# dell-research-harvard/effocr

Hardware: AMD Instinct MI355X
Metric: glyph-crops/sec end-to-end (encode+kNN), 224x224 bs=1024 (higher is better)
Workload: dtype bf16; 1 GPU; BASELINE configs[1]: vit_small_patch16_224 encoder (bf16 MFMA operands, fp32 accumulate/residual/LN/softmax), 1024x3x224x224 fp32 crops per GPU resident in HBM, 10000-row fp32 IndexFlatIP, k=10; seeded random-init weights; crops_per_gpu=1024, global_batch=1024, index_rows=10000, k=10, parallelism=1024 crops per GPU, weights+index replicated

## Files before the change

effocr_amd/csrc/qkvattn.hip:

```cpp
#include "common.hpp"
#include "kernels.hpp"
#include <math.h>
#include <type_traits>

#ifndef QA_NT
#define QA_NT 0
#endif
#ifndef QA_ODD_TILE_WAVE
#define QA_ODD_TILE_WAVE 1
#endif
#ifndef QA_BARRIER_DRAIN
#define QA_BARRIER_DRAIN 0
#endif
#ifndef QA_EDGE_BLOCK_MAJOR
#define QA_EDGE_BLOCK_MAJOR 1
#endif

namespace effocr {
namespace {

#ifdef QA_STAMP
constexpr int QA_STAMP_WGS = 256, QA_STAMP_N = 16;
__device__ unsigned long long qa_stamps[QA_STAMP_WGS * 4 * QA_STAMP_N];
#define QA_STAMP_AT(k) qa_stamps[((blockIdx.x & (QA_STAMP_WGS - 1)) * 4 + w) * QA_STAMP_N + (k)] = __builtin_amdgcn_s_memtime();
#else
#define QA_STAMP_AT(k)
#endif

template <int I, int N, typename F> __device__ __forceinline__ void qa_for(F&& f) {
  if constexpr (I < N) {
    f(std::integral_constant<int, I>{});
    qa_for<I + 1, N>(f);
  }
}


constexpr int QA_STAGE = 16384;
constexpr int QA_RING = 6;

template <typename E, int D, int NTT, bool CLS = false, int NPV = 2 * NTT>
__global__ __launch_bounds__(256, 1) void qkvattn_kernel(QkvAttnArgs a) {
  typedef typename Op16<E>::V8 V8;
  constexpr int HEADS = D / 64;
  constexpr int KC = D / 8;
  constexpr int KT = D / 128;
  constexpr int NSH = 3 * KT;
  constexpr int NS = HEADS * NSH;
  constexpr int NXF = D / 16;
  constexpr int R = QA_RING;
  constexpr bool SMALL = NSH < R - 1;
  static_assert(D % 128 == 0 && NS >= R - 1, "qkvattn: embed dim must be a multiple of 128");
  __shared__ __attribute__((aligned(16))) char smem[R * QA_STAGE + NTT * 8192 + 3 * D * 4];
  char* sK = smem;
  char* sV = sK + NTT * 4096;
  float* sBias = reinterpret_cast<float*>(sV + NTT * 4096);
  char* sW = smem + NTT * 8192 + 3 * D * 4;

  const int tid = threadIdx.x;
  int lane = tid & 63, r31 = lane & 31, half = lane >> 5;
  auto refresh_lane = [&]() __attribute__((always_inline)) {
    asm volatile("" : "+v"(lane));
    r31 = lane & 31;
    half = lane >> 5;
  };
  const int w = wave_id();
  QA_STAMP_AT(14)
  const int T = a.T;
  int64_t tok0 = 0;
  const int HS = a.hsplit > 1 ? a.hsplit : 1, NH = HEADS / HS;
  const int grp = (int)blockIdx.x % HS, slot0 = a.img0 + (int)blockIdx.x / HS, nslots = (int)gridDim.x / HS;
  const int hb = grp * NH;
  const int h0 = ((int)blockIdx.x >> 3) % NH;
  const char* Wb = static_cast<const char*>(a.Wb);

  {
    const unsigned sB_lds = (unsigned)(size_t)(__attribute__((address_space(3))) char*)sBias;
#pragma unroll
    for (int j = 0; j < (3 * D / 4 + 255) / 256; ++j) {
      const int u = j * 256 + tid;
      const char* src = reinterpret_cast<const char*>(a.bias) + (size_t)u * 16;
      const unsigned dst = (unsigned)__builtin_amdgcn_readfirstlane((int)(sB_lds + (unsigned)(j * 256 + (tid >> 6) * 64) * 16u));
      if (u < 3 * D / 4)
        asm volatile("s_mov_b32 m0, %1\n\t"
                     "s_nop 0\n\t"
                     "global_load_lds_dwordx4 %0, off"
                     :: "v"(src), "s"(dst) : "memory", "m0");
    }
  }

  int ih = hb + h0, isec = 0, ikt = 0, islot = 0;
  const unsigned lane16 = (unsigned)(tid & 63) * 16u;
  auto issue_piece = [&](int p) __attribute__((always_inline)) {
    const int rb = (isec * D + ih * 64) / 32 + (w >> 1);
    const __attribute__((address_space(1))) void* src =
        (const __attribute__((address_space(1))) void*)(Wb + ((size_t)rb * KC + ikt * 16 + (w & 1) * 8) * 512 + lane16);
    __attribute__((address_space(3))) void* dst = (__attribute__((address_space(3))) void*)(sW + islot * QA_STAGE + ((w >> 1) * 16 + (w & 1) * 8) * 512);
    switch (p) {
      case 0: __builtin_amdgcn_global_load_lds(src, dst, 16, 0, 0); break;
      case 1: __builtin_amdgcn_global_load_lds(src, dst, 16, 1024, 0); break;
      case 2: __builtin_amdgcn_global_load_lds(src, dst, 16, 2048, 0); break;
      default: __builtin_amdgcn_global_load_lds(src, dst, 16, 3072, 0); break;
    }
  };
  const unsigned sW_lds = (unsigned)(size_t)(__attribute__((address_space(3))) char*)sW;
  auto issue_piece_asm = [&](auto P_) __attribute__((always_inline)) {
    constexpr int pc = decltype(P_)::value;
    const int rb = (isec * D + ih * 64) / 32 + (w >> 1);
    const char* src = Wb + ((size_t)rb * KC + ikt * 16 + (w & 1) * 8) * 512 + lane16;
    const unsigned dst = (unsigned)__builtin_amdgcn_readfirstlane((int)(sW_lds + (unsigned)(islot * QA_STAGE) + (unsigned)(((w >> 1) * 16 + (w & 1) * 8) * 512)));
    unsigned keep;
    asm volatile("s_mov_b32 %0, m0\n\t"
                 "s_mov_b32 m0, %2\n\t"
                 "s_nop 0\n\t"
                 "global_load_lds_dwordx4 %1, off offset:%3\n\t"
                 "s_mov_b32 m0, %0"
                 : "=&s"(keep) : "v"(src), "s"(dst), "n"(pc * 1024) : "memory");
  };
  auto issue_advance = [&]() __attribute__((always_inline)) {
    islot = islot + 1 == R ? 0 : islot + 1;
    if (++ikt == KT) { ikt = 0; if (++isec == 3) { isec = 0; ih = ih + 1 == hb + NH ? hb : ih + 1; } }
  };

  auto run = [&](auto NT_) __attribute__((always_inline)) {
    constexpr int NT = decltype(NT_)::value;
    constexpr int NA = NT > 0 ? NT : 1;
    V8 xf[NA][NXF];

    auto load_frags = [&](int img) __attribute__((always_inline)) {
#pragma unroll
      for (int tt = 0; tt < NT; ++tt) {
        const int t0 = (2 * w + tt) * 32 + r31;
        const int t = t0 < T ? t0 : T - 1;
        const int64_t tok = (int64_t)img * T + t;
        const char* xb = static_cast<const char*>(a.xn) + (tok >> 5) * (int64_t)KC * 512 + (tok & 31) * 16 + half * 512;
#pragma unroll
        for (int i = 0; i < NXF; ++i) {
          xf[tt][i] = (QA_NT & 1) ? __builtin_nontemporal_load(reinterpret_cast<const V8*>(xb + i * 1024)) : *reinterpret_cast<const V8*>(xb + i * 1024);
        }
      }
    };
    const int nimg = (a.B - slot0 + nslots - 1) / nslots;
    const int gtotal = nimg * NH * NSH;
    int slot = 0;
    int g = 0;

    const float cexp = 0.125f * 1.44269504088896340736f;
    constexpr bool INITMASK = NTT > 2;
    f32x16 sinit;
#pragma unroll
    for (int r = 0; r < 16; ++r) sinit[r] = ((NTT - 1) * 32 + (r & 3) + 8 * (r >> 2) + 4 * (lane >> 5) >= T) ? -INFINITY : 0.f;

    auto head = [&](auto LAST_, auto PRE_, int h, int hi, int img_next) __attribute__((always_inline)) {
      constexpr bool LAST = decltype(LAST_)::value;
      constexpr bool PRE = decltype(PRE_)::value;
      refresh_lane();
      QA_STAMP_AT(0)
      V8 qf[NA][4];
      V8 f0, f1;
      constexpr bool EDGE = QA_EDGE_BLOCK_MAJOR && KT >= 2;
      f32x16 acc[NA][2];
      f32x4 hbq[2][2][2];
      float hbv[2];
      float hs[8];
      u32x4 hp;
      auto hand_bias = [&](auto SEC_, auto I_) __attribute__((always_inline)) {
        constexpr int sec = decltype(SEC_)::value, i = decltype(I_)::value;
        if constexpr (sec < 2) {
          const float* bp = sBias + sec * D + h * 64 + i * 32 + 4 * half;
#pragma unroll
          for (int m = 0; m < 2; ++m) {
            hbq[i][m][0] = *reinterpret_cast<const f32x4*>(bp + 8 * (2 * m));
            hbq[i][m][1] = *reinterpret_cast<const f32x4*>(bp + 8 * (2 * m + 1));
          }
        } else {
          hbv[i] = sBias[2 * D + h * 64 + i * 32 + r31];
        }
      };
      u32x2 hlo;
      auto hand_part = [&](auto SEC_, auto I_, auto TT_, auto M_, auto PART_) __attribute__((always_inline)) {
        constexpr int sec = decltype(SEC_)::value, i = decltype(I_)::value, tt = decltype(TT_)::value, m = decltype(M_)::value, part = decltype(PART_)::value;
        if constexpr (part < 2) {
#pragma unroll
          for (int j = 0; j < 4; ++j) {
            if constexpr (sec < 2) hs[4 * part + j] = acc[tt][i][8 * m + 4 * part + j] + hbq[i][m][part][j];
            else hs[4 * part + j] = acc[tt][i][8 * m + 4 * part + j] + hbv[i];
          }
          asm volatile("" : "+v"(hs[4 * part]), "+v"(hs[4 * part + 1]), "+v"(hs[4 * part + 2]), "+v"(hs[4 * part + 3]));
        } else if constexpr (part == 2) {
          hlo = pack4<E>(hs[0], hs[1], hs[2], hs[3]);
          asm volatile("" : "+v"(hlo));
        } else {
          const u32x2 hi = pack4<E>(hs[4], hs[5], hs[6], hs[7]);
          hp = u32x4{hlo[0], hlo[1], hi[0], hi[1]};
          const int tile = 2 * w + tt;
          constexpr bool REAL = QA_ODD_TILE_WAVE && NTT == 7;
          if constexpr (sec == 0) qf[tt][2 * i + m] = __builtin_bit_cast(V8, hp);
          else if (REAL || tile < NTT) {
            if constexpr (sec == 1) *reinterpret_cast<u32x4*>(sK + ((tile * 4 + 2 * i + m) * 64 + lane) * 16) = hp;
            else *reinterpret_cast<u32x4*>(sV + (((tile * 2 + m) * 2 + i) * 64 + lane) * 16) = hp;
          }
        }
      };
      auto hand_block = [&](auto SEC_, auto I_) __attribute__((always_inline)) {
        hand_bias(SEC_, I_);
        qa_for<0, NT>([&](auto TT_) {
          qa_for<0, 2>([&](auto M_) {
            qa_for<0, 4>([&](auto PART_) { hand_part(SEC_, I_, TT_, M_, PART_); });
          });
        });
      };
      qa_for<0, 3>([&](auto SEC_) {
        constexpr int sec = decltype(SEC_)::value;
        if constexpr (!EDGE) {
#pragma unroll
          for (int tt = 0; tt < NA; ++tt)
#pragma unroll
            for (int i = 0; i < 2; ++i)
#pragma unroll
              for (int r = 0; r < 16; ++r) acc[tt][i][r] = 0.f;
        }
        qa_for<0, KT>([&](auto KT_) {
          constexpr int kt = decltype(KT_)::value;
          constexpr int sl = sec * KT + kt;
          constexpr int ft = NSH - 1 - sl;
          constexpr bool BM = EDGE && (kt == 0 || kt == KT - 1);
          constexpr bool NEXT_BM = EDGE && kt + 1 >= KT - 1;
          const char* st = sW + slot * QA_STAGE + half * 512 + r31 * 16;
          const int nslot = slot + 1 == R ? 0 : slot + 1;
          const char* stn = sW + nslot * QA_STAGE + half * 512 + r31 * 16;
          if constexpr (sl == 0) {
            f0 = *reinterpret_cast<const V8*>(st);
            if constexpr (!BM) f1 = *reinterpret_cast<const V8*>(st + 16 * 512);
          }
          auto stage_sync = [&]() __attribute__((always_inline)) {
            if constexpr (SMALL) asm volatile("s_waitcnt vmcnt(0)" ::: "memory");
            else if constexpr (!LAST) asm volatile("s_waitcnt vmcnt(%0)" ::"n"((R - 3) * 4) : "memory");
            else if constexpr (ft >= 1) asm volatile("s_waitcnt vmcnt(%0)" ::"n"(((ft < R - 2 ? ft : R - 2) - 1) * 4) : "memory");
#if QA_BARRIER_DRAIN
            asm volatile("s_waitcnt lgkmcnt(0)" ::: "memory");
#endif
            __builtin_amdgcn_s_barrier();
            asm volatile("" ::: "memory");
          };
          auto stage_piece = [&](auto P_) __attribute__((always_inline)) {
            if constexpr (SMALL) { if (g + R - 1 < gtotal) issue_piece_asm(P_); }
            else if constexpr (!LAST || ft >= R - 1) issue_piece_asm(P_);
          };
          auto mfma_into = [&](auto TT_, auto I_, V8 f, V8 x) __attribute__((always_inline)) {
            constexpr int tt = decltype(TT_)::value, i = decltype(I_)::value;
            if constexpr (sec < 2) return Op16<E>::mfma(f, x, acc[tt][i]);
            else return Op16<E>::mfma(x, f, acc[tt][i]);
          };
          if constexpr (!BM) {
            qa_for<0, 8>([&](auto KS_) {
              constexpr int ks = decltype(KS_)::value;
              if constexpr (ks == 4) stage_sync();
              V8 n0, n1;
              if constexpr (ks < 7) {
                n0 = *reinterpret_cast<const V8*>(st + (2 * (ks + 1)) * 512);
                n1 = *reinterpret_cast<const V8*>(st + (16 + 2 * (ks + 1)) * 512);
              } else if constexpr (sl + 1 < NSH) {
                n0 = *reinterpret_cast<const V8*>(stn);
                if constexpr (!NEXT_BM) n1 = *reinterpret_cast<const V8*>(stn + 16 * 512);
              }
              qa_for<0, NT>([&](auto TT_) {
                constexpr int tt = decltype(TT_)::value;
                if constexpr (CLS && sec == 0) {
                  if (w == 0 && tt == 0) {
                    acc[tt][0] = mfma_into(TT_, std::integral_constant<int, 0>{}, f0, xf[tt][kt * 8 + ks]);
                    acc[tt][1] = mfma_into(TT_, std::integral_constant<int, 1>{}, f1, xf[tt][kt * 8 + ks]);
                  }
                } else {
                  acc[tt][0] = mfma_into(TT_, std::integral_constant<int, 0>{}, f0, xf[tt][kt * 8 + ks]);
                  acc[tt][1] = mfma_into(TT_, std::integral_constant<int, 1>{}, f1, xf[tt][kt * 8 + ks]);
                }
              });
              if constexpr (ks >= 4) stage_piece(std::integral_constant<int, ks - 4>{});
              if constexpr (ks < 7 || sl + 1 < NSH) f0 = n0;
              if constexpr (ks < 7 || (sl + 1 < NSH && !NEXT_BM)) f1 = n1;
            });
          } else {
            constexpr bool HOST_PREV = kt == 0 && sec > 0, HOST_OWN = kt == KT - 1;
            qa_for<0, 2>([&](auto BLK_) {
              constexpr int blk = decltype(BLK_)::value;
              constexpr bool HOSTING = blk == 0 ? HOST_PREV : HOST_OWN;
              qa_for<0, 8>([&](auto KS_) {
                constexpr int ks = decltype(KS_)::value;
                if constexpr (blk == 1 && ks == 0) stage_sync();
                V8 n0, n1;
                if constexpr (ks < 7) n0 = *reinterpret_cast<const V8*>(st + (16 * blk + 2 * (ks + 1)) * 512);
                else if constexpr (blk == 0) n0 = *reinterpret_cast<const V8*>(st + 16 * 512);
                else if constexpr (sl + 1 < NSH) {
                  n0 = *reinterpret_cast<const V8*>(stn);
                  if constexpr (!NEXT_BM) n1 = *reinterpret_cast<const V8*>(stn + 16 * 512);
                }
                qa_for<0, NT>([&](auto TT_) {
                  constexpr int tt = decltype(TT_)::value;
                  if constexpr (kt == 0 && ks == 0) {
#pragma unroll
                    for (int r = 0; r < 16; ++r) acc[tt][blk][r] = 0.f;
                  }
                  if constexpr (CLS && sec == 0) {
                    if (w == 0 && tt == 0) acc[tt][blk] = mfma_into(TT_, BLK_, f0, xf[tt][kt * 8 + ks]);
                  } else {
                    acc[tt][blk] = mfma_into(TT_, BLK_, f0, xf[tt][kt * 8 + ks]);
                  }
                  if constexpr (HOSTING) {
                    constexpr int gi = ks * NT + tt, fr = gi >> 2;
                    __builtin_amdgcn_sched_barrier(0);
                    hand_part(std::integral_constant<int, (blk == 0 ? sec - 1 : sec)>{}, std::integral_constant<int, 1 - blk>{},
                              std::integral_constant<int, (fr >> 1)>{}, std::integral_constant<int, (fr & 1)>{}, std::integral_constant<int, (gi & 3)>{});
                    __builtin_amdgcn_sched_barrier(0);
                  }
                });
                if constexpr (HOST_OWN && ks == 6) {
                  if constexpr (blk == 0) hand_bias(SEC_, std::integral_constant<int, 0>{});
                  else if constexpr (sec < 2) hand_bias(SEC_, std::integral_constant<int, 1>{});
                }
                if constexpr (blk == 1 && (ks & 1) == 0) stage_piece(std::integral_constant<int, ks / 2>{});
                if constexpr (ks < 7 || blk == 0 || sl + 1 < NSH) f0 = n0;
                if constexpr (blk == 1 && ks == 7 && sl + 1 < NSH && !NEXT_BM) f1 = n1;
              });
            });
          }
          if constexpr (SMALL) { if (g + R - 1 < gtotal) issue_advance(); }
          else if constexpr (!LAST || ft >= R - 1) issue_advance();
          slot = slot + 1 == R ? 0 : slot + 1;
          ++g;
        });
        if constexpr (!EDGE) {
          hand_block(SEC_, std::integral_constant<int, 0>{});
          hand_block(SEC_, std::integral_constant<int, 1>{});
        } else if constexpr (sec == 2) {
          hand_block(SEC_, std::integral_constant<int, 1>{});
        }
        QA_STAMP_AT(1 + sec)
      });
      if constexpr (PRE) load_frags(img_next);
      asm volatile("s_waitcnt lgkmcnt(0)" ::: "memory");
      __builtin_amdgcn_s_barrier();
      asm volatile("" ::: "memory");
      QA_STAMP_AT(4)

      const char* kb = sK + lane * 16;
      const char* vb = sV + lane * 16;
      qa_for<0, (CLS ? 1 : NT)>([&](auto TT_) {
        constexpr int tt = decltype(TT_)::value;
        if constexpr (CLS) { if (w != 0) return; }
        if (2 * w + tt >= NTT) return;
        __builtin_amdgcn_sched_barrier(0);
        const int tq = (2 * w + tt) * 32 + r31;
        f32x16 s[NTT];
        constexpr int QA_KDEPTH = 1, KD = QA_KDEPTH + 1;
        V8 kf[KD][4];
#pragma unroll
        for (int d = 0; d < QA_KDEPTH; ++d)
          if (d < NTT) {
#pragma unroll
            for (int ks = 0; ks < 4; ++ks) kf[d][ks] = *reinterpret_cast<const V8*>(kb + (d * 4 + ks) * 1024);
          }
        qa_for<0, NTT>([&](auto KT_) {
          constexpr int kt = decltype(KT_)::value, cur = kt % KD, nxt = (kt + QA_KDEPTH) % KD;
          if constexpr (kt + QA_KDEPTH < NTT) {
#pragma unroll
            for (int ks = 0; ks < 4; ++ks) kf[nxt][ks] = *reinterpret_cast<const V8*>(kb + ((kt + QA_KDEPTH) * 4 + ks) * 1024);
          }
          if constexpr (INITMASK && kt == NTT - 1) s[kt] = sinit;
          else {
#pragma unroll
            for (int r = 0; r < 16; ++r) s[kt][r] = 0.f;
          }
#pragma unroll
          for (int ks = 0; ks < 4; ++ks) s[kt] = Op16<E>::mfma(kf[cur][ks], qf[tt][ks], s[kt]);
          __builtin_amdgcn_sched_barrier(0);
        });
        QA_STAMP_AT(5 + tt * 5)
        V8 vf[2][2];
#pragma unroll
        for (int db = 0; db < 2; ++db) vf[0][db] = *reinterpret_cast<const V8*>(vb + db * 1024);
        float mx = -INFINITY;
#pragma unroll
        for (int kt = 0; kt < NTT; ++kt) {
#pragma unroll
          for (int r = 0; r < 16; ++r) {
            if (!INITMASK) {
              const int key = kt * 32 + (r & 3) + 8 * (r >> 2) + 4 * half;
              if (key >= T) s[kt][r] = -INFINITY;
            }
            mx = fmaxf(mx, s[kt][r]);
          }
        }
        mx = fmaxf(mx, __shfl_xor(mx, 32, 64));
        f32x16 o[2];
#pragma unroll
        for (int db = 0; db < 2; ++db)
#pragma unroll
          for (int r = 0; r < 16; ++r) o[db][r] = 0.f;
        f32x16 lsum;
#pragma unroll
        for (int r = 0; r < 16; ++r) lsum[r] = 0.f;
        const V8 ones = {(E)1.f, (E)1.f, (E)1.f, (E)1.f, (E)1.f, (E)1.f, (E)1.f, (E)1.f};
        const float mxc = mx * cexp;
        __builtin_amdgcn_sched_barrier(0);
        V8 pf[2];
        float av[8], ev[8];
        auto p_part = [&](auto ST_, auto PART_) __attribute__((always_inline)) {
          constexpr int st = decltype(ST_)::value, kt = st >> 1, m = st & 1, part = decltype(PART_)::value;
          if constexpr (part == 0) {
#pragma unroll
            for (int j = 0; j < 4; ++j) av[j] = __builtin_fmaf(s[kt][8 * m + j], cexp, -mxc);
            ev[0] = __builtin_amdgcn_exp2f(av[0]); ev[1] = __builtin_amdgcn_exp2f(av[1]);
          } else if constexpr (part == 1) {
#pragma unroll
            for (int j = 4; j < 8; ++j) av[j] = __builtin_fmaf(s[kt][8 * m + j], cexp, -mxc);
            ev[2] = __builtin_amdgcn_exp2f(av[2]); ev[3] = __builtin_amdgcn_exp2f(av[3]); ev[4] = __builtin_amdgcn_exp2f(av[4]);
          } else {
            ev[5] = __builtin_amdgcn_exp2f(av[5]); ev[6] = __builtin_amdgcn_exp2f(av[6]); ev[7] = __builtin_amdgcn_exp2f(av[7]);
            const u32x4 pw = {pack2<E>(ev[0], ev[1]), pack2<E>(ev[2], ev[3]), pack2<E>(ev[4], ev[5]), pack2<E>(ev[6], ev[7])};
            pf[st & 1] = __builtin_bit_cast(V8, pw);
          }
        };
        QA_STAMP_AT(6 + tt * 5)
        qa_for<0, 3>([&](auto P_) { p_part(std::integral_constant<int, 0>{}, P_); });
        __builtin_amdgcn_sched_barrier(0);
        qa_for<0, NPV>([&](auto ST_) {
          constexpr int st = decltype(ST_)::value, cur = st & 1, nxt = cur ^ 1;
          constexpr bool more = st + 1 < NPV;
          if constexpr (more) {
#pragma unroll
            for (int db = 0; db < 2; ++db) vf[nxt][db] = *reinterpret_cast<const V8*>(vb + ((st + 1) * 2 + db) * 1024);
          }
          o[0] = Op16<E>::mfma(vf[cur][0], pf[cur], o[0]);
          __builtin_amdgcn_sched_barrier(0);
          if constexpr (more) p_part(std::integral_constant<int, st + 1>{}, std::integral_constant<int, 0>{});
          __builtin_amdgcn_sched_barrier(0);
          o[1] = Op16<E>::mfma(vf[cur][1], pf[cur], o[1]);
          __builtin_amdgcn_sched_barrier(0);
          if constexpr (more) p_part(std::integral_constant<int, st + 1>{}, std::integral_constant<int, 1>{});
          __builtin_amdgcn_sched_barrier(0);
          lsum = Op16<E>::mfma(ones, pf[cur], lsum);
          __builtin_amdgcn_sched_barrier(0);
          if constexpr (more) p_part(std::integral_constant<int, st + 1>{}, std::integral_constant<int, 2>{});
          __builtin_amdgcn_sched_barrier(0);
        });
        QA_STAMP_AT(7 + tt * 5)
        const float l = lsum[0];
        if (tq < T) {
          const float inv = 1.0f / l;
          char* ob = static_cast<char*>(a.out);
#pragma unroll
          for (int db = 0; db < 2; ++db)
#pragma unroll
            for (int p = 0; p < 2; ++p) {
              const u32x2 lo = pack4<E>(o[db][8 * p] * inv, o[db][8 * p + 1] * inv, o[db][8 * p + 2] * inv, o[db][8 * p + 3] * inv);
              const u32x2 hi = pack4<E>(o[db][8 * p + 4] * inv, o[db][8 * p + 5] * inv, o[db][8 * p + 6] * inv, o[db][8 * p + 7] * inv);
              const u32x4 v = {lo[0], lo[1], hi[0], hi[1]};
              u32x4* op = reinterpret_cast<u32x4*>(ob + blk_off(tok0 + tq, h * 8 + db * 4 + 2 * p + half, D / 8));
              if (QA_NT & 2) __builtin_nontemporal_store(v, op); else *op = v;
            }
        }
        QA_STAMP_AT(8 + tt * 5)
      });
      QA_STAMP_AT(15)
    };

    load_frags(slot0);
#pragma unroll
    for (int s0 = 0; s0 < R - 1; ++s0) {
#pragma unroll
      for (int p = 0; p < 4; ++p) issue_piece(p);
      issue_advance();
    }
    asm volatile("s_waitcnt vmcnt(%0)" ::"n"((R - 2) * 4) : "memory");
    __builtin_amdgcn_s_barrier();
    asm volatile("" ::: "memory");
#pragma unroll 1
    for (int ii = 0; ii < nimg; ++ii) {
      const int img = slot0 + ii * nslots;
      tok0 = (int64_t)img * T;
      refresh_lane();
#pragma unroll 1
      for (int i = 0; i < NH - 1; ++i) {
        const int h = hb + (h0 + i < NH ? h0 + i : h0 + i - NH);
        head(std::false_type{}, std::false_type{}, h, i, 0);
      }
      const int hl = hb + (h0 == 0 ? NH - 1 : h0 - 1);
      if (ii + 1 < nimg) head(std::false_type{}, std::true_type{}, hl, HEADS - 1, img + nslots);
      else head(std::true_type{}, std::false_type{}, hl, HEADS - 1, 0);
    }
  };

#if QA_ODD_TILE_WAVE
  if ((NTT & 1) && w == 3) run(std::integral_constant<int, 1>{});
  else
#endif
  run(std::integral_constant<int, 2>{});
}

template <typename E>
int launch_qkvattn(const QkvAttnArgs& a, hipStream_t s) {
  const int ntt = (a.T + 31) / 32;
  const int cus = device_cus();
  const int heads = a.D / 64;
  auto split_for = [&](int64_t images) {
    if (a.hsplit == 1 || a.D != 384) return 1;
    for (int c = heads; c >= 2; --c)
      if (heads % c == 0 && images * c <= cus && (a.hsplit <= 0 || c <= a.hsplit)) return c;
    return 1;
  };
  const int64_t nimg_launch = (int64_t)a.B - a.img0;
  int hs = split_for(nimg_launch);
  if (a.img0 == 0 && hs == 1 && a.B > cus && a.hsplit != 1) {
    const int tail = a.B % cus, ths = tail ? split_for(tail) : 1;
    if (ths > 1) {
      QkvAttnArgs m = a, t = a;
      m.B = a.B - tail; m.hsplit = 1;
      t.img0 = a.B - tail;
      const int rc = launch_qkvattn<E>(m, s);
      return rc ? rc : launch_qkvattn<E>(t, s);
    }
  }
  QkvAttnArgs ah = a;
  ah.hsplit = hs;
  const QkvAttnArgs& a2 = ah;
  const dim3 grid((unsigned)(hs > 1 ? nimg_launch * hs : (nimg_launch < cus ? nimg_launch : cus))), blk(256);
  const bool short_tail = a.T <= 32 * ntt - 16;
  if (a.D == 384 && ntt == 7 && a.cls_only && short_tail) hipLaunchKernelGGL((qkvattn_kernel<E, 384, 7, true, 13>), grid, blk, 0, s, a2);
  else if (a.D == 384 && ntt == 7 && a.cls_only) hipLaunchKernelGGL((qkvattn_kernel<E, 384, 7, true>), grid, blk, 0, s, a2);
  else if (a.D == 384 && ntt == 7 && short_tail) hipLaunchKernelGGL((qkvattn_kernel<E, 384, 7, false, 13>), grid, blk, 0, s, a2);
  else if (a.D == 384 && ntt == 7) hipLaunchKernelGGL((qkvattn_kernel<E, 384, 7>), grid, blk, 0, s, a2);
  else if (a.D == 384 && ntt <= 2) hipLaunchKernelGGL((qkvattn_kernel<E, 384, 2>), grid, blk, 0, s, a2);
  else if (a.D == 128 && ntt == 7) hipLaunchKernelGGL((qkvattn_kernel<E, 128, 7>), grid, blk, 0, s, a2);
  else if (a.D == 128 && ntt <= 2) hipLaunchKernelGGL((qkvattn_kernel<E, 128, 2>), grid, blk, 0, s, a2);
  else return fail(EFFOCR_EUNSUPPORTED, "qkv_attn_fused: (embed dim, tokens) must be (128|384, <=64 or 193..224)");
  return check_launch("qkv_attn_fused");
}

}

bool qkv_attn_supported(int prec, int D, int T) {
  const int ntt = (T + 31) / 32;
  return prec != PREC_FP32 && (D == 384 || D == 128) && T >= 1 && (ntt <= 2 || ntt == 7);
}

int qkv_attn_fused(int prec, const QkvAttnArgs& a, hipStream_t s) {
  if (a.B <= 0) return EFFOCR_OK;
  if (!qkv_attn_supported(prec, a.D, a.T)) return fail(EFFOCR_EUNSUPPORTED, "qkv_attn_fused: unsupported (precision, embed dim, tokens)");
  if (a.rows_alloc % 32 || a.rows_alloc < (int64_t)a.B * a.T) return fail(EFFOCR_EINVAL, "qkv_attn_fused: rows_alloc must be a multiple of 32 >= batch * tokens");
  if ((reinterpret_cast<uintptr_t>(a.bias) & 15) != 0) return fail(EFFOCR_EINVAL, "qkv_attn_fused: the bias array must be 16-byte aligned (it reaches LDS by 16-byte DMA)");
  return prec == PREC_BF16 ? launch_qkvattn<__bf16>(a, s) : launch_qkvattn<_Float16>(a, s);
}


}

#ifdef QA_STAMP
extern "C" int effocr_debug_qa_stamps(unsigned long long* out, int n) {
  const int m = effocr::QA_STAMP_WGS * 4 * effocr::QA_STAMP_N;
  if (n < m) return -1;
  return hipMemcpyFromSymbol(out, HIP_SYMBOL(effocr::qa_stamps), (size_t)m * 8) == hipSuccess ? 0 : -2;
}
#endif
```

Measured before the change: 95860 glyph-crops/s.

## Defer attention output epilogue and interleave it with next MFMA streams

For the 7-tile (T=197) case, the attention output normalisation, bf16 packing and global store are deferred. They are split into 17 slices and interleaved between MFMAs: the first query tile's epilogue runs inside the second tile's QK^T MFMAs, and the last tile's epilogue runs inside the next head's QKV projection MFMAs. The aim is to hide the VALU and store latency of the epilogue behind matrix work. In exchange it keeps extra live registers (po, d_o) across phases, which raises VGPR pressure. It also adds a tail flush after the loop and removes the early-return for the odd tile.

After: 96490 glyph-crops/s, median of 6. About the same (+0.7%).

```diff
diff --git a/effocr_amd/csrc/qkvattn.hip b/effocr_amd/csrc/qkvattn.hip
--- a/effocr_amd/csrc/qkvattn.hip
+++ b/effocr_amd/csrc/qkvattn.hip
@@ -15,12 +15,15 @@
 #ifndef QA_EDGE_BLOCK_MAJOR
 #define QA_EDGE_BLOCK_MAJOR 1
 #endif
+#ifndef QA_EPILOGUE_HOSTED
+#define QA_EPILOGUE_HOSTED 1
+#endif
 
 namespace effocr {
 namespace {
 
 #ifdef QA_STAMP
-constexpr int QA_STAMP_WGS = 256, QA_STAMP_N = 16;
+constexpr int QA_STAMP_WGS = 256, QA_STAMP_N = 24;
 __device__ unsigned long long qa_stamps[QA_STAMP_WGS * 4 * QA_STAMP_N];
 #define QA_STAMP_AT(k) qa_stamps[((blockIdx.x & (QA_STAMP_WGS - 1)) * 4 + w) * QA_STAMP_N + (k)] = __builtin_amdgcn_s_memtime();
 #else
@@ -149,6 +152,45 @@
     f32x16 sinit;
 #pragma unroll
     for (int r = 0; r < 16; ++r) sinit[r] = ((NTT - 1) * 32 + (r & 3) + 8 * (r >> 2) + 4 * (lane >> 5) >= T) ? -INFINITY : 0.f;
+
+    constexpr bool HOSTED = QA_EPILOGUE_HOSTED && QA_EDGE_BLOCK_MAJOR && QA_ODD_TILE_WAVE && KT >= 2 && !CLS && NTT == 7;
+    constexpr int EPI_SLICES = 17;
+    f32x16 po[2];
+    float pl = 1.f;
+    int ptq = T, ph = 0;
+    int64_t ptok0 = 0;
+    if constexpr (HOSTED) {
+#pragma unroll
+      for (int db = 0; db < 2; ++db)
+#pragma unroll
+        for (int r = 0; r < 16; ++r) po[db][r] = 0.f;
+    }
+    float einv, es[8];
+    u32x2 elo;
+    auto epi_part = [&](auto S_, const f32x16 (&eo)[2], float el, int etq, int64_t etok0, int eh) __attribute__((always_inline)) {
+      constexpr int sl = decltype(S_)::value;
+      if constexpr (sl == 0) {
+        einv = 1.0f / el;
+        asm volatile("" : "+v"(einv));
+      } else {
+        constexpr int fr = (sl - 1) >> 2, part = (sl - 1) & 3, db = fr >> 1, p = fr & 1;
+        if constexpr (part < 2) {
+#pragma unroll
+          for (int j = 0; j < 4; ++j) es[4 * part + j] = eo[db][8 * p + 4 * part + j] * einv;
+          asm volatile("" : "+v"(es[4 * part]), "+v"(es[4 * part + 1]), "+v"(es[4 * part + 2]), "+v"(es[4 * part + 3]));
+        } else if constexpr (part == 2) {
+          elo = pack4<E>(es[0], es[1], es[2], es[3]);
+          asm volatile("" : "+v"(elo));
+        } else {
+          const u32x2 ehi = pack4<E>(es[4], es[5], es[6], es[7]);
+          const u32x4 v = {elo[0], elo[1], ehi[0], ehi[1]};
+          if (etq < T) {
+            u32x4* op = reinterpret_cast<u32x4*>(static_cast<char*>(a.out) + blk_off(etok0 + etq, eh * 8 + db * 4 + 2 * p + half, D / 8));
+            if (QA_NT & 2) __builtin_nontemporal_store(v, op); else *op = v;
+          }
+        }
+      }
+    };
 
     auto head = [&](auto LAST_, auto PRE_, int h, int hi, int img_next) __attribute__((always_inline)) {
       constexpr bool LAST = decltype(LAST_)::value;
@@ -305,6 +347,15 @@
                   } else {
                     acc[tt][blk] = mfma_into(TT_, BLK_, f0, xf[tt][kt * 8 + ks]);
                   }
+                  if constexpr (HOSTED && sec == 0 && kt == 0) {
+                    constexpr int gi = (blk * 8 + ks) * NT + tt;
+                    if constexpr (gi < EPI_SLICES) {
+                      __builtin_amdgcn_sched_barrier(0);
+                      epi_part(std::integral_constant<int, gi>{}, po, pl, ptq, ptok0, ph);
+                      if constexpr (gi + 1 == 16 * NT && gi + 1 < EPI_SLICES) epi_part(std::integral_constant<int, gi + 1>{}, po, pl, ptq, ptok0, ph);
+                      __builtin_amdgcn_sched_barrier(0);
+                    }
+                  }
                   if constexpr (HOSTING) {
                     constexpr int gi = ks * NT + tt, fr = gi >> 2;
                     __builtin_amdgcn_sched_barrier(0);
@@ -327,6 +378,7 @@
           else if constexpr (!LAST || ft >= R - 1) issue_advance();
           slot = slot + 1 == R ? 0 : slot + 1;
           ++g;
+          if constexpr (sl == 0) { QA_STAMP_AT(16) }
         });
         if constexpr (!EDGE) {
           hand_block(SEC_, std::integral_constant<int, 0>{});
@@ -344,10 +396,13 @@
 
       const char* kb = sK + lane * 16;
       const char* vb = sV + lane * 16;
+      f32x16 d_o[2];
+      float d_l = 1.f;
       qa_for<0, (CLS ? 1 : NT)>([&](auto TT_) {
         constexpr int tt = decltype(TT_)::value;
+        constexpr bool HOST_T0 = HOSTED && tt == 1;
         if constexpr (CLS) { if (w != 0) return; }
-        if (2 * w + tt >= NTT) return;
+        if constexpr (!HOSTED) { if (2 * w + tt >= NTT) return; }
         __builtin_amdgcn_sched_barrier(0);
         const int tq = (2 * w + tt) * 32 + r31;
         f32x16 s[NTT];
@@ -370,8 +425,24 @@
 #pragma unroll
             for (int r = 0; r < 16; ++r) s[kt][r] = 0.f;
           }
-#pragma unroll
-          for (int ks = 0; ks < 4; ++ks) s[kt] = Op16<E>::mfma(kf[cur][ks], qf[tt][ks], s[kt]);
+          if constexpr (HOST_T0) {
+            if constexpr (kt == 0) {
+              epi_part(std::integral_constant<int, 0>{}, d_o, d_l, (2 * w) * 32 + r31, tok0, h);
+              __builtin_amdgcn_sched_barrier(0);
+            }
+            qa_for<0, 4>([&](auto KS_) {
+              constexpr int ks = decltype(KS_)::value, gi = kt * 4 + ks;
+              s[kt] = Op16<E>::mfma(kf[cur][ks], qf[tt][ks], s[kt]);
+              if constexpr (gi + 1 < EPI_SLICES) {
+                __builtin_amdgcn_sched_barrier(0);
+                epi_part(std::integral_constant<int, gi + 1>{}, d_o, d_l, (2 * w) * 32 + r31, tok0, h);
+                __builtin_amdgcn_sched_barrier(0);
+              }
+            });
+          } else {
+#pragma unroll
+            for (int ks = 0; ks < 4; ++ks) s[kt] = Op16<E>::mfma(kf[cur][ks], qf[tt][ks], s[kt]);
+          }
           __builtin_amdgcn_sched_barrier(0);
         });
         QA_STAMP_AT(5 + tt * 5)
@@ -445,7 +516,14 @@
         });
         QA_STAMP_AT(7 + tt * 5)
         const float l = lsum[0];
-        if (tq < T) {
+        if constexpr (HOSTED) {
+          if constexpr (tt + 1 < NT) {
+            d_o[0] = o[0]; d_o[1] = o[1]; d_l = l;
+          } else {
+            po[0] = o[0]; po[1] = o[1]; pl = l;
+            ptq = tq; ptok0 = tok0; ph = h;
+          }
+        } else if (tq < T) {
           const float inv = 1.0f / l;
           char* ob = static_cast<char*>(a.out);
 #pragma unroll
@@ -487,6 +565,10 @@
       const int hl = hb + (h0 == 0 ? NH - 1 : h0 - 1);
       if (ii + 1 < nimg) head(std::false_type{}, std::true_type{}, hl, HEADS - 1, img + nslots);
       else head(std::true_type{}, std::false_type{}, hl, HEADS - 1, 0);
+    }
+    if constexpr (HOSTED) {
+      refresh_lane();
+      qa_for<0, EPI_SLICES>([&](auto S_) { epi_part(S_, po, pl, ptq, ptok0, ph); });
     }
   };
 
@@ -555,6 +637,10 @@
 }
 
 #ifdef QA_STAMP
+extern "C" int effocr_debug_qa_layout(int* hosted) {
+  if (hosted) *hosted = QA_EPILOGUE_HOSTED && QA_EDGE_BLOCK_MAJOR && QA_ODD_TILE_WAVE;
+  return effocr::QA_STAMP_N;
+}
 extern "C" int effocr_debug_qa_stamps(unsigned long long* out, int n) {
   const int m = effocr::QA_STAMP_WGS * 4 * effocr::QA_STAMP_N;
   if (n < m) return -1;
```
